# cscott/compressjs

Measured on NVIDIA H100. Metric: bzip2_-9_encode_MBps, higher is better.
Workload: dtype u8

## Files before the change

compressjs_b200/csrc/rle1.cu:

```cuda
#include <algorithm>
#include <cstdlib>
#include "enc.h"

#define RT_THREADS 256
#define RT_PER 16

struct TileSum {
  u32 lead, trail, rest;
  u8 fc, lc, allsame, pad;
};

__host__ __device__ __forceinline__ u64 outfresh(u64 c) {
  u64 q = c / 255, r = c % 255;
  return 5 * q + (r <= 3 ? r : 5);
}
__host__ __device__ __forceinline__ u64 cneed(u64 target) {
  u64 q = (target - 1) / 5, rem = target - 5 * q;
  return 255 * q + (rem <= 3 ? rem : 4);
}
__device__ __forceinline__ u32 w_of_dist(u32 d) {
  u32 r = d % 255 + 1;
  return r <= 3 ? 1u : (r == 4 ? 2u : 0u);
}

struct TileView {
  u8 by[RT_PER];
  u8 w[RT_PER];
  u32 cnt;
  u32 excl;
  u32 total;
  u32 first_start;
  u32 last_start;
  u32 len;
};

struct TileScratch {
  u32 ws[RT_THREADS / 32 + 1];
  u8 lastb[RT_THREADS];
  u32 red[RT_THREADS / 32];
};

__device__ __forceinline__ u32 block_excl_max256(u32 v, u32* ws) {
  u32 inc = warp_incl_max(v);
  u32 exw = __shfl_up_sync(FULL_MASK, inc, 1);
  if (lane_id() == 0) exw = 0;
  const int w = threadIdx.x >> 5;
  if (lane_id() == 31) ws[w] = inc;
  __syncthreads();
  if (w == 0) {
    u32 x = (lane_id() < RT_THREADS / 32) ? ws[lane_id()] : 0u;
    u32 xi = warp_incl_max(x);
    u32 xe = __shfl_up_sync(FULL_MASK, xi, 1);
    if (lane_id() == 0) xe = 0;
    if (lane_id() < RT_THREADS / 32) ws[lane_id()] = xe;
  }
  __syncthreads();
  u32 c = ws[w];
  __syncthreads();
  return exw > c ? exw : c;
}
__device__ __forceinline__ u32 block_min256(u32 v, u32* red) {
#pragma unroll
  for (int o = 16; o > 0; o >>= 1) v = min(v, __shfl_xor_sync(FULL_MASK, v, o));
  if (lane_id() == 0) red[threadIdx.x >> 5] = v;
  __syncthreads();
  u32 r = red[0];
#pragma unroll
  for (int i = 1; i < RT_THREADS / 32; i++) r = min(r, red[i]);
  __syncthreads();
  return r;
}
__device__ __forceinline__ u32 block_max256(u32 v, u32* red) {
#pragma unroll
  for (int o = 16; o > 0; o >>= 1) v = max(v, __shfl_xor_sync(FULL_MASK, v, o));
  if (lane_id() == 0) red[threadIdx.x >> 5] = v;
  __syncthreads();
  u32 r = red[0];
#pragma unroll
  for (int i = 1; i < RT_THREADS / 32; i++) r = max(r, red[i]);
  __syncthreads();
  return r;
}

__device__ void tile_view(const u8* __restrict__ in, u64 N, u64 tstart, u32 carry, TileScratch& sc, TileView& v) {
  const u32 tid = threadIdx.x;
  const u64 remain = N - tstart;
  v.len = remain < RLE_TILE ? (u32)remain : RLE_TILE;
  const u32 pos0 = tid * RT_PER;
  v.cnt = pos0 >= v.len ? 0 : min((u32)RT_PER, v.len - pos0);
  const u8* p = in + tstart + pos0;
  if (v.cnt == RT_PER && (((size_t)p) & 15) == 0) {
    uint4 q = *reinterpret_cast<const uint4*>(p);
    u32 a[4] = {q.x, q.y, q.z, q.w};
#pragma unroll
    for (int j = 0; j < RT_PER; j++) v.by[j] = (u8)(a[j >> 2] >> ((j & 3) * 8));
  } else {
#pragma unroll
    for (int j = 0; j < RT_PER; j++) v.by[j] = (j < (int)v.cnt) ? p[j] : 0;
  }
  sc.lastb[tid] = v.by[RT_PER - 1];
  __syncthreads();
  const u8 prev0 = tid ? sc.lastb[tid - 1] : 0;
  u32 smask = 0, last_local = 0, first_local = 0xffffffffu;
#pragma unroll
  for (int j = 0; j < RT_PER; j++) {
    if (j < (int)v.cnt) {
      const u32 pos = pos0 + j;
      const u8 pb = j ? v.by[j - 1] : prev0;
      const bool st = (pos == 0) || (v.by[j] != pb);
      if (st) {
        smask |= 1u << j;
        last_local = pos + 1;
        if (pos > 0 && first_local == 0xffffffffu) first_local = pos;
      }
    }
  }
  const u32 ex = block_excl_max256(last_local, sc.ws);
  u32 rs = ex ? ex - 1 : 0;
  u32 sum = 0;
#pragma unroll
  for (int j = 0; j < RT_PER; j++) {
    u32 ww = 0;
    if (j < (int)v.cnt) {
      const u32 pos = pos0 + j;
      if (smask & (1u << j)) rs = pos;
      const u32 d = pos - rs + (rs == 0 ? carry : 0);
      ww = w_of_dist(d);
    }
    v.w[j] = (u8)ww;
    sum += ww;
  }
  u32 total;
  v.excl = block_excl_add<RT_THREADS, u32>(sum, sc.ws, &total);
  v.total = total;
  u32 fs = block_min256(first_local, sc.red);
  v.first_start = fs == 0xffffffffu ? v.len : fs;
  u32 ls = block_max256(last_local, sc.red);
  v.last_start = ls ? ls - 1 : 0;
}

__global__ void __launch_bounds__(RT_THREADS) k_rle_summary(const u8* __restrict__ in, u64 N, TileSum* __restrict__ sums, u8* __restrict__ plain) {
  __shared__ TileScratch sc;
  __shared__ u32 lastw[RT_THREADS];
  const u64 t = blockIdx.x;
  const u64 tstart = t * RLE_TILE;
  const u32 tid = threadIdx.x;
  const u64 remain = N - tstart;
  const u32 len = remain < RLE_TILE ? (u32)remain : RLE_TILE;
  const u8* p = in + tstart + tid * RT_PER;
  if (len == RLE_TILE && ((((size_t)in) + tstart) & 15) == 0) {
    const uint4 q = *reinterpret_cast<const uint4*>(p);
    lastw[tid] = q.w;
    __syncthreads();
    u32 prevw;
    if (tid) prevw = lastw[tid - 1];
    else if (tstart >= 4) prevw = ((u32)in[tstart - 1] << 24) | ((u32)in[tstart - 2] << 16) | ((u32)in[tstart - 3] << 8);
    else {
      prevw = 0;
      for (int k = 1; k <= 3; k++) {
        const u32 b = (tstart >= (u64)k) ? in[tstart - k] : (u32)((u8)(~q.x) + k);
        prevw |= b << (8 * (4 - k));
      }
    }
    const u32 a[5] = {prevw, q.x, q.y, q.z, q.w};
    u32 any4 = 0;
#pragma unroll
    for (int wv = 1; wv < 5; wv++) {
      const u32 cur = a[wv], sh1 = __funnelshift_l(a[wv - 1], cur, 8);
      const u32 sh2 = __funnelshift_l(a[wv - 1], cur, 16), sh3 = __funnelshift_l(a[wv - 1], cur, 24);
      const u32 e = __vcmpeq4(cur, sh1) & __vcmpeq4(cur, sh2) & __vcmpeq4(cur, sh3);
      any4 |= e;
    }
    if (!__syncthreads_or(any4 != 0)) {
      if (tid == 0) {
        TileSum s;
        s.fc = in[tstart];
        s.lc = in[tstart + len - 1];
        u32 lead = 1;
        while (lead < 4 && in[tstart + lead] == s.fc) lead++;
        u32 trail = 1;
        while (trail < 4 && in[tstart + len - 1 - trail] == s.lc) trail++;
        s.lead = lead; s.trail = trail; s.allsame = 0; s.rest = len - lead; s.pad = 0;
        sums[t] = s;
        plain[t] = 1;
      }
      return;
    }
  }
  TileView v;
  tile_view(in, N, tstart, 0, sc, v);
  if (threadIdx.x == 0) {
    plain[t] = 0;
    TileSum s;
    s.fc = in[tstart];
    s.lc = in[tstart + v.len - 1];
    s.lead = v.first_start;
    s.allsame = v.first_start == v.len;
    s.trail = v.len - v.last_start;
    s.rest = v.total - (u32)outfresh(v.first_start);
    s.pad = 0;
    sums[t] = s;
  }
}

__device__ __forceinline__ u64 rs_make(bool allsame, u32 fc, u32 lc, u32 trail, u32 len) {
  return (1ull << 63) | ((u64)allsame << 62) | ((u64)fc << 24) | ((u64)lc << 16) | ((u64)trail << 8) | (u64)len;
}
__device__ __forceinline__ u64 rs_combine(u64 A, u64 B) {
  if (!(A >> 63)) return B;
  if (!(B >> 63)) return A;
  const bool Aall = (A >> 62) & 1, Ball = (B >> 62) & 1;
  const u32 Afc = (A >> 24) & 255, Alc = (A >> 16) & 255, Atr = (A >> 8) & 255, Alen = A & 255;
  const u32 Bfc = (B >> 24) & 255, Blc = (B >> 16) & 255, Btr = (B >> 8) & 255, Blen = B & 255;
  const bool join = Alc == Bfc;
  const u32 trail = (Ball && join) ? (Atr + Blen) % 255 : Btr;
  return rs_make(Aall && Ball && join, Afc, Blc, trail, (Alen + Blen) % 255);
}

#define RS_THREADS 1024
__global__ void __launch_bounds__(RS_THREADS)
k_rle_scan(const TileSum* __restrict__ sums, u64 ntiles, u64 N, u32* __restrict__ carry, u64* __restrict__ prefix, u64 st0, u64 W0,
           u64* __restrict__ agg_out) {
  __shared__ u64 sa[RS_THREADS], sb[RS_THREADS];
  const u32 tid = threadIdx.x;
  const u64 per = (ntiles + RS_THREADS - 1) / RS_THREADS;
  const u64 t0 = (u64)tid * per, t1 = min(ntiles, t0 + per);
  u64 agg = 0;
  for (u64 t = t0; t < t1; t++) {
    const TileSum s = sums[t];
    const u64 tl = min((u64)RLE_TILE, N - t * RLE_TILE);
    agg = rs_combine(agg, rs_make(s.allsame, s.fc, s.lc, s.trail % 255, (u32)(tl % 255)));
  }
  sa[tid] = agg;
  __syncthreads();
  u64* src = sa; u64* dst = sb;
  for (u32 o = 1; o < RS_THREADS; o <<= 1) {
    u64 x = src[tid];
    if (tid >= o) x = rs_combine(src[tid - o], x);
    dst[tid] = x;
    __syncthreads();
    u64* tmp = src; src = dst; dst = tmp;
  }
  u64 st = rs_combine(st0, tid ? src[tid - 1] : 0);
  if (tid == 0 && agg_out) *agg_out = src[RS_THREADS - 1];
  __syncthreads();
  u64 mysum = 0;
  for (u64 t = t0; t < t1; t++) {
    const TileSum s = sums[t];
    const u64 tl = min((u64)RLE_TILE, N - t * RLE_TILE);
    u32 c = 0;
    if ((st >> 63) && ((st >> 16) & 255) == s.fc) c = (st >> 8) & 255;
    carry[t] = c;
    const u64 S = outfresh((u64)c + s.lead) - outfresh(c) + s.rest;
    prefix[t] = S;
    mysum += S;
    st = rs_combine(st, rs_make(s.allsame, s.fc, s.lc, s.trail % 255, (u32)(tl % 255)));
  }
  sa[tid] = mysum;
  __syncthreads();
  src = sa; dst = sb;
  for (u32 o = 1; o < RS_THREADS; o <<= 1) {
    u64 x = src[tid];
    if (tid >= o) x += src[tid - o];
    dst[tid] = x;
    __syncthreads();
    u64* tmp = src; src = dst; dst = tmp;
  }
  u64 run = W0 + (tid ? src[tid - 1] : 0);
  const u64 grand = W0 + src[RS_THREADS - 1];
  for (u64 t = t0; t < t1; t++) {
    const u64 S = prefix[t];
    prefix[t] = run;
    run += S;
  }
  if (tid == 0) prefix[ntiles] = grand;
}

#define RG_THREADS 256
#define RG_PER 8
#define RG_TILES (RG_THREADS * RG_PER)
__device__ __forceinline__ u64 rg_tile_state(const TileSum& s, u64 t, u64 N) {
  const u64 tl = min((u64)RLE_TILE, N - t * RLE_TILE);
  return rs_make(s.allsame, s.fc, s.lc, s.trail % 255, (u32)(tl % 255));
}
__device__ __forceinline__ u64 rg_block_excl_state(u64 v, u64* sa, u64* sb, u64* total) {
  const u32 tid = threadIdx.x;
  sa[tid] = v;
  __syncthreads();
  u64* src = sa; u64* dst = sb;
  for (u32 o = 1; o < RG_THREADS; o <<= 1) {
    u64 x = src[tid];
    if (tid >= o) x = rs_combine(src[tid - o], x);
    dst[tid] = x;
    __syncthreads();
    u64* tmp = src; src = dst; dst = tmp;
  }
  const u64 ex = tid ? src[tid - 1] : 0;
  *total = src[RG_THREADS - 1];
  __syncthreads();
  return ex;
}
__global__ void __launch_bounds__(RG_THREADS)
k_rle_scan_g1(const TileSum* __restrict__ sums, u64 ntiles, u64 N, u64* __restrict__ group_agg) {
  __shared__ u64 sa[RG_THREADS], sb[RG_THREADS];
  const u64 t0 = (u64)blockIdx.x * RG_TILES + (u64)threadIdx.x * RG_PER;
  u64 agg = 0;
  for (u32 j = 0; j < RG_PER; j++) {
    const u64 t = t0 + j;
    if (t < ntiles) agg = rs_combine(agg, rg_tile_state(sums[t], t, N));
  }
  u64 total;
  rg_block_excl_state(agg, sa, sb, &total);
  if (threadIdx.x == 0) group_agg[blockIdx.x] = total;
}
template <bool STATE>
__global__ void __launch_bounds__(RS_THREADS)
k_rle_scan_groups(const u64* __restrict__ in, u32 ngroups, u64* __restrict__ out, u64 init, u64* __restrict__ agg_out) {
  __shared__ u64 sa[RS_THREADS], sb[RS_THREADS];
  const u32 tid = threadIdx.x;
  const u32 per = (ngroups + RS_THREADS - 1) / RS_THREADS;
  const u32 g0 = tid * per, g1 = min(ngroups, g0 + per);
  u64 agg = 0;
  for (u32 g = g0; g < g1; g++) agg = STATE ? rs_combine(agg, in[g]) : agg + in[g];
  sa[tid] = agg;
  __syncthreads();
  u64* src = sa; u64* dst = sb;
  for (u32 o = 1; o < RS_THREADS; o <<= 1) {
    u64 x = src[tid];
    if (tid >= o) x = STATE ? rs_combine(src[tid - o], x) : src[tid - o] + x;
    dst[tid] = x;
    __syncthreads();
    u64* tmp = src; src = dst; dst = tmp;
  }
  u64 run = tid ? src[tid - 1] : 0;
  run = STATE ? rs_combine(init, run) : init + run;
  if (tid == 0 && agg_out) *agg_out = src[RS_THREADS - 1];
  for (u32 g = g0; g < g1; g++) {
    const u64 v = in[g];
    out[g] = run;
    run = STATE ? rs_combine(run, v) : run + v;
  }
  if (tid == RS_THREADS - 1) out[ngroups] = STATE ? rs_combine(init, src[RS_THREADS - 1]) : init + src[RS_THREADS - 1];
}
__global__ void __launch_bounds__(RG_THREADS)
k_rle_scan_g3(const TileSum* __restrict__ sums, u64 ntiles, u64 N, const u64* __restrict__ group_start, u32* __restrict__ carry,
              u64* __restrict__ prefix, u64* __restrict__ group_sum) {
  __shared__ u64 sa[RG_THREADS], sb[RG_THREADS];
  __shared__ u32 ws[RG_THREADS / 32 + 1];
  const u64 t0 = (u64)blockIdx.x * RG_TILES + (u64)threadIdx.x * RG_PER;
  TileSum ts[RG_PER];
  u64 agg = 0;
#pragma unroll
  for (u32 j = 0; j < RG_PER; j++) {
    const u64 t = t0 + j;
    if (t < ntiles) { ts[j] = sums[t]; agg = rs_combine(agg, rg_tile_state(ts[j], t, N)); }
  }
  u64 total;
  u64 st = rs_combine(group_start[blockIdx.x], rg_block_excl_state(agg, sa, sb, &total));
  u32 mysum = 0;
#pragma unroll
  for (u32 j = 0; j < RG_PER; j++) {
    const u64 t = t0 + j;
    if (t < ntiles) {
      const TileSum& s = ts[j];
      u32 c = 0;
      if ((st >> 63) && ((st >> 16) & 255) == s.fc) c = (st >> 8) & 255;
      carry[t] = c;
      const u64 S = outfresh((u64)c + s.lead) - outfresh(c) + s.rest;
      prefix[t] = S;
      mysum += (u32)S;
      st = rs_combine(st, rg_tile_state(s, t, N));
    }
  }
  u32 tot;
  block_excl_add<RG_THREADS, u32>(mysum, ws, &tot);
  if (threadIdx.x == 0) group_sum[blockIdx.x] = tot;
}
__global__ void __launch_bounds__(RG_THREADS)
k_rle_scan_g5(u64 ntiles, const u64* __restrict__ group_base, u32 ngroups, u64* __restrict__ prefix) {
  __shared__ u32 ws[RG_THREADS / 32 + 1];
  const u64 t0 = (u64)blockIdx.x * RG_TILES + (u64)threadIdx.x * RG_PER;
  u32 S[RG_PER];
  u32 mysum = 0;
#pragma unroll
  for (u32 j = 0; j < RG_PER; j++) {
    const u64 t = t0 + j;
    S[j] = t < ntiles ? (u32)prefix[t] : 0u;
    mysum += S[j];
  }
  u32 tot;
  u64 run = group_base[blockIdx.x] + block_excl_add<RG_THREADS, u32>(mysum, ws, &tot);
#pragma unroll
  for (u32 j = 0; j < RG_PER; j++) {
    const u64 t = t0 + j;
    if (t < ntiles) { prefix[t] = run; run += S[j]; }
  }
  if (blockIdx.x == 0 && threadIdx.x == 0) prefix[ntiles] = group_base[ngroups];
}

struct BlocksShared {
  TileScratch sc;
  u64 r64;
  u32 r32;
};

__device__ u64 eval_W(const u8* in, u64 N, const u32* carry, const u64* prefix, u64 x, BlocksShared& sh) {
  const u64 t = x / RLE_TILE;
  const u32 off = (u32)(x % RLE_TILE);
  if (off == 0) return prefix[t];
  TileView v;
  tile_view(in, N, t * RLE_TILE, carry[t], sh.sc, v);
  const u32 tid = threadIdx.x;
  if (off / RT_PER == tid) {
    u32 a = v.excl;
    for (u32 j = 0; j < off % RT_PER; j++) a += v.w[j];
    sh.r64 = prefix[t] + a;
  }
  __syncthreads();
  u64 r = sh.r64;
  __syncthreads();
  return r;
}

__device__ u64 find_run_end(const u8* in, u64 s, u64 cap, BlocksShared& sh) {
  const u8 ch = in[s];
  for (u64 base = s; base < cap; base += RLE_TILE) {
    const u64 p0 = base + (u64)threadIdx.x * RT_PER;
    u32 found = 0xffffffffu;
    for (u32 j = 0; j < RT_PER; j++) {
      const u64 p = p0 + j;
      if (p < cap && in[p] != ch) { found = (u32)(p - base); break; }
    }
    const u32 f = block_min256(found, sh.sc.red);
    if (f != 0xffffffffu) return base + f;
  }
  return cap;
}

__global__ void __launch_bounds__(RT_THREADS)
k_rle_blocks(const u8* __restrict__ in, u64 N, u32 BS, const u32* __restrict__ carry, const u64* __restrict__ prefix, u64 ntiles,
             BlkInfo* __restrict__ blocks, u32* nblocks_out, u32 maxblocks, u64 u_start, u32 range_first, u32 range_count, int open_end) {
  __shared__ BlocksShared sh;
  const u32 tid = threadIdx.x;
  const u64 Wtotal = prefix[ntiles];
  if (gridDim.x > 1) {
    const u32 P = gridDim.x, r = blockIdx.x;
    const u32 first = range_first + (u32)((u64)r * range_count / P), next = range_first + (u32)((u64)(r + 1) * range_count / P);
    u_start = (u64)first * BS;
    blocks += first - range_first;
    nblocks_out += r;
    maxblocks = (r == P - 1 && open_end) ? maxblocks - (first - range_first) : next - first;
  }
  u64 s = 0, Ws = prefix[0];
  bool Ws_valid = true;
  u32 k = 0;
  if (u_start > 0) {
    if (u_start > Wtotal) { if (tid == 0) *nblocks_out = 0; return; }
    u64 lo = 0, hi = ntiles;
    while (hi - lo > 1) {
      const u64 span = hi - lo;
      const u64 pi = lo + 1 + (span - 1) * (u64)tid / RT_THREADS;
      const bool valid = pi < hi && (tid == 0 || pi != lo + 1 + (span - 1) * (u64)(tid - 1) / RT_THREADS);
      const bool pr = valid && prefix[pi] < u_start;
      const u32 tr = block_max256(pr ? tid + 1 : 0, sh.sc.red);
      const u32 fl = block_min256((valid && !pr) ? tid : 0xffffffffu, sh.sc.red);
      u64 nlo = lo, nhi = hi;
      if (tr) nlo = lo + 1 + (span - 1) * (u64)(tr - 1) / RT_THREADS;
      if (fl != 0xffffffffu) nhi = lo + 1 + (span - 1) * (u64)fl / RT_THREADS;
      lo = nlo; hi = nhi;
    }
    const u64 t = lo;
    TileView v;
    tile_view(in, N, t * RLE_TILE, carry[t], sh.sc, v);
    u32 found = 0xffffffffu;
    {
      u64 acc = prefix[t] + v.excl;
      for (u32 j = 0; j < v.cnt; j++) {
        acc += v.w[j];
        if (acc >= u_start) { found = tid * RT_PER + j; break; }
      }
    }
    const u32 f = block_min256(found, sh.sc.red);
    if (f / RT_PER == tid) {
      u64 acc = prefix[t] + v.excl;
      for (u32 j = 0; j <= f % RT_PER; j++) acc += v.w[j];
      sh.r64 = acc;
    }
    __syncthreads();
    Ws = sh.r64;
    __syncthreads();
    s = t * RLE_TILE + f + 1;
    Ws_valid = true;
  }
  while (s < N && k < maxblocks) {
    BlkInfo bi;
    bi.s = s;
    const bool midrun = s > 0 && in[s - 1] == in[s];
    u64 b = s;
    if (midrun) {
      const u64 cap = min(N, s + cneed(BS));
      b = find_run_end(in, s, cap, sh);
    }
    const u64 ofs = outfresh(b - s);
    u64 e;
    if (ofs >= BS) {
      e = s + cneed(BS);
      bi.e = e; bi.b = e; bi.Wb = 0; bi.ofs = 0; bi.n = BS;
      Ws_valid = false;
    } else {
      u64 Wb;
      if (midrun) Wb = eval_W(in, N, carry, prefix, b, sh);
      else Wb = Ws_valid ? Ws : eval_W(in, N, carry, prefix, s, sh);
      const u64 V = Wb + (BS - ofs);
      if (V > Wtotal) {
        e = N;
        bi.e = e; bi.b = b; bi.Wb = Wb; bi.ofs = (u32)ofs; bi.n = (u32)(ofs + (Wtotal - Wb));
        Ws_valid = false;
      } else {
        u64 lo = b / RLE_TILE, hi = ntiles;
        {
          const u64 plo = prefix[lo];
          u64 tg = lo + ((V - plo) >> 12);
          if (tg >= ntiles) tg = ntiles - 1;
          const u64 pg = prefix[tg], pg1 = prefix[tg + 1];
          if (pg < V && pg1 >= V) { lo = tg; hi = tg + 1; }
          else if (pg < V) lo = tg;
          else if (tg > lo) hi = tg;
        }
        if (hi - lo > 1) {
          const u64 a = ((BS - ofs) * 4 / 5) / RLE_TILE;
          const u64 g0 = lo + (a > 1 ? a - 1 : 0);
          if (g0 < ntiles && prefix[g0] < V) {
            lo = g0;
            const u64 g1 = g0 + 4 * RT_THREADS;
            if (g1 < ntiles && !(prefix[g1] < V)) hi = g1;
          }
        }
        while (hi - lo > 1) {
          const u64 span = hi - lo;
          const u64 pi = lo + 1 + (span - 1) * (u64)tid / RT_THREADS;
          const bool valid = pi < hi && (tid == 0 || pi != lo + 1 + (span - 1) * (u64)(tid - 1) / RT_THREADS);
          const bool pr = valid && prefix[pi] < V;
          const u32 tr = block_max256(pr ? tid + 1 : 0, sh.sc.red);
          const u32 fl = block_min256((valid && !pr) ? tid : 0xffffffffu, sh.sc.red);
          u64 nlo = lo, nhi = hi;
          if (tr) nlo = lo + 1 + (span - 1) * (u64)(tr - 1) / RT_THREADS;
          if (fl != 0xffffffffu) nhi = lo + 1 + (span - 1) * (u64)fl / RT_THREADS;
          lo = nlo; hi = nhi;
        }
        const u64 t = lo;
        TileView v;
        tile_view(in, N, t * RLE_TILE, carry[t], sh.sc, v);
        u32 found = 0xffffffffu;
        {
          u64 acc = prefix[t] + v.excl;
          for (u32 j = 0; j < v.cnt; j++) {
            acc += v.w[j];
            if (acc >= V) { found = tid * RT_PER + j; break; }
          }
        }
        const u32 f = block_min256(found, sh.sc.red);
        if (f / RT_PER == tid) {
          u64 acc = prefix[t] + v.excl;
          for (u32 j = 0; j <= f % RT_PER; j++) acc += v.w[j];
          sh.r64 = acc;
        }
        __syncthreads();
        const u64 We = sh.r64;
        __syncthreads();
        e = t * RLE_TILE + f + 1;
        const u64 produced = ofs + (We - Wb);
        bi.e = e; bi.b = b; bi.Wb = Wb; bi.ofs = (u32)ofs; bi.n = (u32)min(produced, (u64)BS);
        Ws = We; Ws_valid = true;
      }
    }
    if (tid == 0) blocks[k] = bi;
    k++;
    s = e;
  }
  if (tid == 0) *nblocks_out = k;
}

__global__ void __launch_bounds__(RT_THREADS)
k_rle_emit(const u8* __restrict__ in, u64 N, const u32* __restrict__ carry, const u64* __restrict__ prefix, const u8* __restrict__ plain,
           const BlkInfo* __restrict__ blocks, u32 first, u32 count, const u64* __restrict__ tile_base, u8* __restrict__ T) {
  __shared__ TileScratch sc;
  __shared__ u32 s_k;
  __shared__ __align__(16) u8 stage[RLE_TILE + 32];
  if (threadIdx.x == 0) {
    u32 lo = 0, hi = count;
    while (hi - lo > 1) {
      u32 mid = (lo + hi) >> 1;
      if (tile_base[mid] <= blockIdx.x) lo = mid; else hi = mid;
    }
    s_k = lo;
  }
  __syncthreads();
  const u32 kk = s_k;
  const BlkInfo bi = blocks[first + kk];
  const u64 t = bi.s / RLE_TILE + (blockIdx.x - tile_base[kk]);
  const u64 tstart = t * RLE_TILE;
  u8* Tb = T + ((size_t)kk << SEG_SHIFT);
  const u64 Pt = prefix[t];
  if (plain[t]) {
    const u64 remain = N - tstart;
    const u32 len = remain < RLE_TILE ? (u32)remain : RLE_TILE;
    const u64 x0 = bi.s > tstart ? bi.s : tstart;
    const u64 x1 = (bi.e < tstart + len) ? bi.e : tstart + len;
    if (x0 >= x1) return;
    const u64 o0 = x0 < bi.b ? (x0 - bi.s) : (u64)bi.ofs + (Pt + (x0 - tstart) - bi.Wb);
    if (o0 >= bi.n) return;
    const u32 cnt = (u32)min((u64)(x1 - x0), (u64)bi.n - o0);
    const u32 fo = (u32)(o0 & 15u);
    const u8* src = in + x0;
    for (u32 i = threadIdx.x * 16u; i < cnt; i += RT_THREADS * 16u) {
      if (i + 16u <= cnt && ((((size_t)src) + i) & 15u) == 0) {
        const uint4 q = *reinterpret_cast<const uint4*>(src + i);
        const u32 a[4] = {q.x, q.y, q.z, q.w};
#pragma unroll
        for (int j = 0; j < 16; j++) stage[fo + i + j] = (u8)(a[j >> 2] >> ((j & 3) * 8));
      } else {
        const u32 e = min(i + 16u, cnt);
        for (u32 x = i; x < e; x++) stage[fo + x] = src[x];
      }
    }
    __syncthreads();
    const u32 last = fo + cnt;
    u8* dst = Tb + (o0 - fo);
    for (u32 c16 = threadIdx.x * 16u; c16 < last; c16 += RT_THREADS * 16u) {
      if (c16 >= fo && c16 + 16u <= last) *reinterpret_cast<uint4*>(dst + c16) = *reinterpret_cast<const uint4*>(stage + c16);
      else {
        const u32 e = min(c16 + 16u, last);
        for (u32 x = max(c16, fo); x < e; x++) dst[x] = stage[x];
      }
    }
    return;
  }
  TileView v;
  tile_view(in, N, tstart, carry[t], sc, v);
  u32 run = v.excl;
  for (u32 j = 0; j < v.cnt; j++) {
    const u64 x = tstart + threadIdx.x * RT_PER + j;
    const u32 wmax = v.w[j];
    const u32 exw = run;
    run += wmax;
    if (x < bi.s || x >= bi.e) continue;
    u32 r;
    u64 opos;
    if (x < bi.b) {
      const u64 d = x - bi.s;
      r = (u32)(d % 255) + 1;
      opos = outfresh(d);
    } else {
      r = wmax == 0 ? 5u : (wmax == 2 ? 4u : 1u);
      opos = bi.ofs + (Pt + exw - bi.Wb);
    }
    if (r > 4 || opos >= bi.n) continue;
    const u8 ch = v.by[j];
    Tb[opos] = ch;
    if (r == 4 && opos + 1 < bi.n) {
      u64 lim = x + 1 + 251;
      if (lim > bi.e) lim = bi.e;
      if (x < bi.b && lim > bi.b) lim = bi.b;
      u32 c = 0;
      while (x + 1 + c < lim && in[x + 1 + c] == ch) c++;
      Tb[opos + 1] = (u8)c;
    }
  }
}

#define CRC_POLY 0x04c11db7u
__host__ __device__ __forceinline__ u32 gf_mulmod(u32 a, u32 b) {
  u32 r = 0;
  for (int i = 31; i >= 0; i--) {
    r = (r << 1) ^ ((r & 0x80000000u) ? CRC_POLY : 0u);
    if ((b >> i) & 1) r ^= a;
  }
  return r;
}
struct CrcConsts {
  u32 table[256];
  u32 pow[48];
  u32 slice[3][256];
};
static CrcConsts make_crc_consts() {
  CrcConsts c;
  for (u32 i = 0; i < 256; i++) {
    u32 v = i << 24;
    for (int k = 0; k < 8; k++) v = (v & 0x80000000u) ? (v << 1) ^ CRC_POLY : (v << 1);
    c.table[i] = v;
  }
  for (int k = 0; k < 3; k++)
    for (u32 i = 0; i < 256; i++) {
      const u32 prev = k ? c.slice[k - 1][i] : c.table[i];
      c.slice[k][i] = (prev << 8) ^ c.table[prev >> 24];
    }
  c.pow[0] = 0x100;
  for (int i = 1; i < 48; i++) c.pow[i] = gf_mulmod(c.pow[i - 1], c.pow[i - 1]);
  return c;
}
__constant__ CrcConsts c_crc;
static bool g_crc_ready = false;
static void crc_setup() {
  if (g_crc_ready) return;
  CrcConsts h = make_crc_consts();
  CUDA_CHECK(cudaMemcpyToSymbol(c_crc, &h, sizeof h));
  g_crc_ready = true;
}
__device__ __forceinline__ u32 crc_xpow(u64 bytes) {
  u32 r = 1u;
  for (int i = 0; bytes; i++, bytes >>= 1)
    if (bytes & 1) r = gf_mulmod(r, c_crc.pow[i]);
  return r;
}

#define CRC_PIECE 256
__host__ __device__ __forceinline__ u64 crc_piece_count(u64 s, u64 e, u32 mis) {
  return e > s ? (e - 1 + mis) / CRC_PIECE - (s + mis) / CRC_PIECE + 1 : 0;
}
__global__ void __launch_bounds__(256)
k_crc_pieces(const u8* __restrict__ in, const BlkInfo* __restrict__ blocks, u32 first, u32 count, const u64* __restrict__ piece_base,
             u64 total_pieces, u32* __restrict__ acc) {
  __shared__ u32 tab[256], t1[256], t2[256], t3[256];
  tab[threadIdx.x] = c_crc.table[threadIdx.x];
  t1[threadIdx.x] = c_crc.slice[0][threadIdx.x];
  t2[threadIdx.x] = c_crc.slice[1][threadIdx.x];
  t3[threadIdx.x] = c_crc.slice[2][threadIdx.x];
  __syncthreads();
  const u64 gid = (u64)blockIdx.x * blockDim.x + threadIdx.x;
  if (gid >= total_pieces) return;
  u32 lo = 0, hi = count;
  while (hi - lo > 1) {
    u32 mid = (lo + hi) >> 1;
    if (piece_base[mid] <= gid) lo = mid; else hi = mid;
  }
  const BlkInfo bi = blocks[first + lo];
  const u32 mis = (u32)((size_t)in & (CRC_PIECE - 1));
  const u64 j = gid - piece_base[lo];
  const u64 A = ((bi.s + mis) / CRC_PIECE + j) * CRC_PIECE;
  const u64 pbeg = A > bi.s + mis ? A - mis : bi.s;
  const u64 pend = A + CRC_PIECE < bi.e + mis ? A + CRC_PIECE - mis : bi.e;
  u32 crc = 0;
  const u8* p = in + pbeg;
  const u32 len = (u32)(pend - pbeg);
  if (len == CRC_PIECE) {
    for (u32 i = 0; i < CRC_PIECE; i += 16) {
      uint4 q = *reinterpret_cast<const uint4*>(p + i);
      u32 a[4] = {q.x, q.y, q.z, q.w};
#pragma unroll
      for (int w = 0; w < 4; w++) {
        const u32 x = crc ^ __byte_perm(a[w], 0, 0x0123);
        crc = t3[x >> 24] ^ t2[(x >> 16) & 0xff] ^ t1[(x >> 8) & 0xff] ^ tab[x & 0xff];
      }
    }
  } else {
    for (u32 i = 0; i < len; i++) crc = (crc << 8) ^ tab[((crc >> 24) ^ p[i]) & 0xff];
  }
  if (pend == bi.e) {
    atomicXor(&acc[2 * lo + 1], crc);
  } else {
    const u64 k = (bi.e - pend) / CRC_PIECE;
    if (k) crc = gf_mulmod(crc, crc_xpow(k * CRC_PIECE));
    atomicXor(&acc[2 * lo], crc);
  }
}
__global__ void k_crc_final(const u8* __restrict__ in, const BlkInfo* __restrict__ blocks, u32 first, u32 count, const u32* __restrict__ acc,
                            u32* __restrict__ crc_out) {
  u32 k = blockIdx.x * blockDim.x + threadIdx.x;
  if (k >= count) return;
  const BlkInfo bi = blocks[first + k];
  const u64 len = bi.e - bi.s;
  const u32 mis = (u32)((size_t)in & (CRC_PIECE - 1));
  const u32 body = gf_mulmod(acc[2 * k], crc_xpow((bi.e + mis) % CRC_PIECE)) ^ acc[2 * k + 1];
  crc_out[k] = ~(body ^ gf_mulmod(0xffffffffu, crc_xpow(len)));
}

u32 crc32_device(Ctx& c, const u8* d_p, size_t n) {
  crc_setup();
  BlkInfo bi;
  memset(&bi, 0, sizeof bi);
  bi.s = 0; bi.e = n; bi.b = 0; bi.n = 0;
  DBuf<BlkInfo> db(c, 1);
  DBuf<u64> pb(c, 1);
  DBuf<u32> acc(c, 2), out(c, 1);
  u64 zero = 0;
  c.to_device(db, &bi, sizeof bi);
  c.to_device(pb, &zero, 8);
  CUDA_CHECK(cudaMemsetAsync(acc, 0, 8, c.stream));
  const u64 pieces = crc_piece_count(0, n, (u32)((size_t)d_p & (CRC_PIECE - 1)));
  if (pieces) {
    k_crc_pieces<<<(unsigned)((pieces + 255) / 256), 256, 0, c.stream>>>(d_p, db, 0, 1, pb, pieces, acc);
    KLAUNCH(c); KCHECK();
  }
  k_crc_final<<<1, 32, 0, c.stream>>>(d_p, db, 0, 1, acc, out);
  KLAUNCH(c); KCHECK();
  u32 h = 0;
  c.to_host(&h, out, 4);
  c.sync();
  return h;
}

__global__ void k_share_lead(const TileSum* __restrict__ sums, u64 ntiles, u64* __restrict__ out) {
  if (threadIdx.x) return;
  u64 lead = 0;
  const u8 fc = sums[0].fc;
  for (u64 t = 0; t < ntiles; t++) {
    const TileSum s = sums[t];
    if (s.fc != fc) break;
    lead += s.lead;
    if (!s.allsame) break;
  }
  *out = lead;
}

void rle1_scan_tiles(Ctx& c, const u8* d_in, size_t n, Rle1Plan& plan, u64 st0, u64 W0, u64* summary) {
  crc_setup();
  StageScope s(c, ST_RLE1);
  if (n == 0) return;
  const u64 ntiles = (n + RLE_TILE - 1) / RLE_TILE;
  DBuf<TileSum> sums(c, ntiles);
  DBuf<u64> dagg(c, 4);
  plan.tile_carry.alloc(c, ntiles);
  plan.tile_prefix.alloc(c, ntiles + 1);
  plan.tile_plain.alloc(c, ntiles);
  k_rle_summary<<<(unsigned)ntiles, RT_THREADS, 0, c.stream>>>(d_in, n, sums, plan.tile_plain);
  KLAUNCH(c); KCHECK();
  static const bool force_groups = getenv("B2_RLE_SCAN_GROUPS") != nullptr;
  if (ntiles <= 4 * RG_TILES && !force_groups) {
    k_rle_scan<<<1, RS_THREADS, 0, c.stream>>>(sums, ntiles, n, plan.tile_carry, plan.tile_prefix, st0, W0, dagg);
    KLAUNCH(c); KCHECK();
  } else {
    c.stats.rle_group_scans++;
    const u32 ng = (u32)((ntiles + RG_TILES - 1) / RG_TILES);
    DBuf<u64> gagg(c, ng), gstart(c, ng + 1), gsum(c, ng), gbase(c, ng + 1);
    k_rle_scan_g1<<<ng, RG_THREADS, 0, c.stream>>>(sums, ntiles, n, gagg);
    KLAUNCH(c); KCHECK();
    k_rle_scan_groups<true><<<1, RS_THREADS, 0, c.stream>>>(gagg, ng, gstart, st0, dagg);
    KLAUNCH(c); KCHECK();
    k_rle_scan_g3<<<ng, RG_THREADS, 0, c.stream>>>(sums, ntiles, n, gstart, plan.tile_carry, plan.tile_prefix, gsum);
    KLAUNCH(c); KCHECK();
    k_rle_scan_groups<false><<<1, RS_THREADS, 0, c.stream>>>(gsum, ng, gbase, W0, nullptr);
    KLAUNCH(c); KCHECK();
    k_rle_scan_g5<<<ng, RG_THREADS, 0, c.stream>>>(ntiles, gbase, ng, plan.tile_prefix);
    KLAUNCH(c); KCHECK();
  }
  if (summary) {
    k_share_lead<<<1, 32, 0, c.stream>>>(sums, ntiles, dagg.p + 1);
    KLAUNCH(c); KCHECK();
    c.to_host(summary, dagg, 16);
  }
  c.to_host(&plan.w_total, plan.tile_prefix.p + ntiles, 8);
  c.sync();
}

static void cut_blocks(Ctx& c, const u8* d_in, size_t n, int level, Rle1Plan& plan, bool exact, size_t first, size_t count) {
  StageScope s(c, ST_RLE1);
  if (n == 0) return;
  const u32 BS = rle1_block_size(level);
  const u64 ntiles = (n + RLE_TILE - 1) / RLE_TILE;
  u32 maxblocks = (u32)(n / ((u64)BS * 4 / 5) + 2);
  u64 u_start = 0;
  if (!exact) {
    maxblocks = (u32)std::min<size_t>(maxblocks, count);
    u_start = (u64)first * BS;
    plan.first_index = first;
    if (maxblocks == 0) return;
  }
  plan.blocks.alloc(c, maxblocks);
  const u32 total = (u32)plan.total_guess(level);
  const u32 rfirst = exact ? 0u : (u32)first, rcount = exact ? total : maxblocks;
  const u32 P = std::min<u32>(64, rcount / 8);
  if (P > 1 && (!exact || total < maxblocks)) {
    DBuf<u32> dnb(c, P);
    k_rle_blocks<<<P, RT_THREADS, 0, c.stream>>>(d_in, n, BS, plan.tile_carry, plan.tile_prefix, ntiles, plan.blocks, dnb, maxblocks, 0, rfirst, rcount,
                                                exact ? 1 : 0);
    KLAUNCH(c); KCHECK();
    std::vector<u32> cut(P);
    c.to_host(cut.data(), dnb, 4 * P);
    c.sync();
    bool ok = true;
    for (u32 r = 0; r + 1 < P && ok; r++) ok = cut[r] == (u32)((u64)(r + 1) * rcount / P) - (u32)((u64)r * rcount / P);
    const u32 last_first = (u32)((u64)(P - 1) * rcount / P);
    ok = ok && cut[P - 1] > 0;
    if (ok) {
      const u32 nb = last_first + cut[P - 1];
      plan.h_blocks.resize(nb);
      c.to_host(plan.h_blocks.data(), plan.blocks, sizeof(BlkInfo) * nb);
      c.sync();
      ok = !exact || (plan.h_blocks[0].s == 0 && plan.h_blocks[nb - 1].e == n);
      for (u32 k = 0; k + 1 < nb && ok; k++) ok = plan.h_blocks[k].e == plan.h_blocks[k + 1].s;
      if (ok) { plan.nblocks = nb; c.stats.rle_walk_parallel++; return; }
      plan.h_blocks.clear();
    }
  }
  c.stats.rle_walk_serial++;
  DBuf<u32> dnb(c, 1);
  k_rle_blocks<<<1, RT_THREADS, 0, c.stream>>>(d_in, n, BS, plan.tile_carry, plan.tile_prefix, ntiles, plan.blocks, dnb, maxblocks, u_start, 0, 0, 0);
  KLAUNCH(c); KCHECK();
  u32 nb = 0;
  c.to_host(&nb, dnb, 4);
  c.sync();
  plan.nblocks = nb;
  plan.h_blocks.resize(nb);
  if (nb) c.to_host(plan.h_blocks.data(), plan.blocks, sizeof(BlkInfo) * nb);
  c.sync();
}
void rle1_cut_range(Ctx& c, const u8* d_in, size_t n, int level, Rle1Plan& plan, size_t first, size_t count) {
  cut_blocks(c, d_in, n, level, plan, false, first, count);
}
void rle1_plan(Ctx& c, const u8* d_in, size_t n, int level, Rle1Plan& plan) {
  rle1_scan_tiles(c, d_in, n, plan);
  cut_blocks(c, d_in, n, level, plan, true, 0, 0);
}
void rle1_materialize(Ctx& c, const u8* d_in, size_t n, const Rle1Plan& plan, size_t first, size_t count, u8* d_T, u32* d_n, u32* d_crc) {
  if (count == 0) return;
  std::vector<u64> tbase(count + 1), pbase(count + 1);
  std::vector<u32> hn(count);
  u64 tt = 0, pp = 0;
  for (size_t k = 0; k < count; k++) {
    const BlkInfo& bi = plan.h_blocks[first + k];
    tbase[k] = tt; pbase[k] = pp;
    tt += (bi.e - 1) / RLE_TILE - bi.s / RLE_TILE + 1;
    pp += crc_piece_count(bi.s, bi.e, (u32)((size_t)d_in & (CRC_PIECE - 1)));
    hn[k] = bi.n;
  }
  tbase[count] = tt; pbase[count] = pp;
  DBuf<u64> dtb(c, count + 1), dpb(c, count + 1);
  DBuf<u32> acc(c, 2 * count);
  c.to_device(dtb, tbase.data(), 8 * (count + 1));
  c.to_device(dpb, pbase.data(), 8 * (count + 1));
  c.to_device(d_n, hn.data(), 4 * count);
  CUDA_CHECK(cudaMemsetAsync(acc, 0, 8 * count, c.stream));
  k_rle_emit<<<(unsigned)tt, RT_THREADS, 0, c.stream>>>(d_in, n, plan.tile_carry, plan.tile_prefix, plan.tile_plain, plan.blocks, (u32)first, (u32)count, dtb, d_T);
  KLAUNCH(c); KCHECK();
  k_crc_pieces<<<(unsigned)((pp + 255) / 256), 256, 0, c.stream>>>(d_in, plan.blocks, (u32)first, (u32)count, dpb, pp, acc);
  KLAUNCH(c); KCHECK();
  k_crc_final<<<(unsigned)((count + 127) / 128), 128, 0, c.stream>>>(d_in, plan.blocks, (u32)first, (u32)count, acc, d_crc);
  KLAUNCH(c); KCHECK();
}

void crc_ranges(Ctx& c, const u8* d_data, const BlkInfo* d_ranges, const std::vector<BlkInfo>& h_ranges, u32* d_crc_out) {
  crc_setup();
  const size_t count = h_ranges.size();
  if (count == 0) return;
  std::vector<u64> pbase(count + 1);
  u64 pp = 0;
  for (size_t k = 0; k < count; k++) {
    pbase[k] = pp;
    pp += crc_piece_count(h_ranges[k].s, h_ranges[k].e, (u32)((size_t)d_data & (CRC_PIECE - 1)));
  }
  pbase[count] = pp;
  DBuf<u64> dpb(c, count + 1);
  DBuf<u32> acc(c, 2 * count);
  c.to_device(dpb, pbase.data(), 8 * (count + 1));
  CUDA_CHECK(cudaMemsetAsync(acc, 0, 8 * count, c.stream));
  if (pp) {
    k_crc_pieces<<<(unsigned)((pp + 255) / 256), 256, 0, c.stream>>>(d_data, d_ranges, 0, (u32)count, dpb, pp, acc);
    KLAUNCH(c); KCHECK();
  }
  k_crc_final<<<(unsigned)((count + 127) / 128), 128, 0, c.stream>>>(d_data, d_ranges, 0, (u32)count, acc, d_crc_out);
  KLAUNCH(c); KCHECK();
  c.sync();
}
```

Before: 25340.

## Fuse block CRC into RLE1 emit kernel with multi-tile spans

The RLE1 emit kernel now handles four tiles per CTA, stages the input bytes in swizzled shared memory, and computes the block CRC from that staged data using segment CRCs combined through precomputed GF(2) power tables. This replaces the separate k_crc_pieces pass over the input, and the device-side binary search is replaced by a precomputed block/span map. The cost is a larger constant table in global memory, an extra small map kernel, more shared memory per CTA, and a hard limit on block length.

```diff
diff --git a/compressjs_b200/csrc/rle1.cu b/compressjs_b200/csrc/rle1.cu
--- a/compressjs_b200/csrc/rle1.cu
+++ b/compressjs_b200/csrc/rle1.cu
@@ -581,63 +581,112 @@
   if (tid == 0) *nblocks_out = k;
 }
 
-__global__ void __launch_bounds__(RT_THREADS)
-k_rle_emit(const u8* __restrict__ in, u64 N, const u32* __restrict__ carry, const u64* __restrict__ prefix, const u8* __restrict__ plain,
-           const BlkInfo* __restrict__ blocks, u32 first, u32 count, const u64* __restrict__ tile_base, u8* __restrict__ T) {
-  __shared__ TileScratch sc;
-  __shared__ u32 s_k;
-  __shared__ __align__(16) u8 stage[RLE_TILE + 32];
-  if (threadIdx.x == 0) {
-    u32 lo = 0, hi = count;
-    while (hi - lo > 1) {
-      u32 mid = (lo + hi) >> 1;
-      if (tile_base[mid] <= blockIdx.x) lo = mid; else hi = mid;
-    }
-    s_k = lo;
-  }
-  __syncthreads();
-  const u32 kk = s_k;
-  const BlkInfo bi = blocks[first + kk];
-  const u64 t = bi.s / RLE_TILE + (blockIdx.x - tile_base[kk]);
-  const u64 tstart = t * RLE_TILE;
-  u8* Tb = T + ((size_t)kk << SEG_SHIFT);
-  const u64 Pt = prefix[t];
-  if (plain[t]) {
-    const u64 remain = N - tstart;
-    const u32 len = remain < RLE_TILE ? (u32)remain : RLE_TILE;
-    const u64 x0 = bi.s > tstart ? bi.s : tstart;
-    const u64 x1 = (bi.e < tstart + len) ? bi.e : tstart + len;
-    if (x0 >= x1) return;
-    const u64 o0 = x0 < bi.b ? (x0 - bi.s) : (u64)bi.ofs + (Pt + (x0 - tstart) - bi.Wb);
-    if (o0 >= bi.n) return;
-    const u32 cnt = (u32)min((u64)(x1 - x0), (u64)bi.n - o0);
-    const u32 fo = (u32)(o0 & 15u);
-    const u8* src = in + x0;
-    for (u32 i = threadIdx.x * 16u; i < cnt; i += RT_THREADS * 16u) {
-      if (i + 16u <= cnt && ((((size_t)src) + i) & 15u) == 0) {
-        const uint4 q = *reinterpret_cast<const uint4*>(src + i);
-        const u32 a[4] = {q.x, q.y, q.z, q.w};
-#pragma unroll
-        for (int j = 0; j < 16; j++) stage[fo + i + j] = (u8)(a[j >> 2] >> ((j & 3) * 8));
-      } else {
-        const u32 e = min(i + 16u, cnt);
-        for (u32 x = i; x < e; x++) stage[fo + x] = src[x];
-      }
-    }
-    __syncthreads();
-    const u32 last = fo + cnt;
-    u8* dst = Tb + (o0 - fo);
-    for (u32 c16 = threadIdx.x * 16u; c16 < last; c16 += RT_THREADS * 16u) {
-      if (c16 >= fo && c16 + 16u <= last) *reinterpret_cast<uint4*>(dst + c16) = *reinterpret_cast<const uint4*>(stage + c16);
-      else {
-        const u32 e = min(c16 + 16u, last);
-        for (u32 x = max(c16, fo); x < e; x++) dst[x] = stage[x];
-      }
-    }
-    return;
-  }
-  TileView v;
-  tile_view(in, N, tstart, carry[t], sc, v);
+#define CRC_POLY 0x04c11db7u
+__host__ __device__ __forceinline__ u32 gf_mulmod(u32 a, u32 b) {
+  u32 r = 0;
+  for (int i = 31; i >= 0; i--) {
+    r = (r << 1) ^ ((r & 0x80000000u) ? CRC_POLY : 0u);
+    if ((b >> i) & 1) r ^= a;
+  }
+  return r;
+}
+#define EMIT_TILES 4
+#define EMIT_SPAN (EMIT_TILES * RLE_TILE)
+#define EMIT_SEG 64
+static_assert(EMIT_SEG * RT_THREADS == EMIT_SPAN, "every emit thread takes one segment of the span");
+#define CRC_TILE_POWS 11264
+struct CrcConsts {
+  u32 slice[4][256];
+  u32 pow[48];
+  u32 pow_byte[EMIT_SEG + 1];
+  u32 pow_seg[EMIT_SPAN / EMIT_SEG];
+  u32 pow_tile[CRC_TILE_POWS];
+};
+static void make_crc_consts(CrcConsts& c) {
+  for (u32 i = 0; i < 256; i++) {
+    u32 v = i << 24;
+    for (int k = 0; k < 8; k++) v = (v & 0x80000000u) ? (v << 1) ^ CRC_POLY : (v << 1);
+    c.slice[0][i] = v;
+  }
+  for (int k = 1; k < 4; k++)
+    for (u32 i = 0; i < 256; i++) {
+      const u32 prev = c.slice[k - 1][i];
+      c.slice[k][i] = (prev << 8) ^ c.slice[0][prev >> 24];
+    }
+  c.pow[0] = 0x100;
+  for (int i = 1; i < 48; i++) c.pow[i] = gf_mulmod(c.pow[i - 1], c.pow[i - 1]);
+  c.pow_byte[0] = 1u;
+  for (int r = 1; r <= EMIT_SEG; r++) c.pow_byte[r] = gf_mulmod(c.pow_byte[r - 1], c.pow[0]);
+  c.pow_seg[0] = 1u;
+  for (int m = 1; m < EMIT_SPAN / EMIT_SEG; m++) c.pow_seg[m] = gf_mulmod(c.pow_seg[m - 1], c.pow_byte[EMIT_SEG]);
+  const u32 xtile = c.pow[12];
+  c.pow_tile[0] = 1u;
+  for (int k = 1; k < CRC_TILE_POWS; k++) c.pow_tile[k] = gf_mulmod(c.pow_tile[k - 1], xtile);
+}
+static_assert(RLE_TILE == 1 << 12, "pow_tile is built from pow[12]");
+__device__ CrcConsts g_crc;
+static bool g_crc_ready = false;
+static void crc_setup() {
+  if (g_crc_ready) return;
+  static CrcConsts h;
+  make_crc_consts(h);
+  CUDA_CHECK(cudaMemcpyToSymbol(g_crc, &h, sizeof h));
+  g_crc_ready = true;
+}
+__device__ __forceinline__ u32 crc_xpow(u64 bytes) {
+  u32 r = 1u;
+  for (int i = 0; bytes; i++, bytes >>= 1)
+    if (bytes & 1) r = gf_mulmod(r, g_crc.pow[i]);
+  return r;
+}
+__device__ __forceinline__ void crc_load_tables(u32 (*tab)[256]) {
+#pragma unroll
+  for (int k = 0; k < 4; k++) tab[k][threadIdx.x] = g_crc.slice[k][threadIdx.x];
+}
+__device__ __forceinline__ u32 crc_step4(u32 crc, u32 w, const u32 (*tab)[256]) {
+  const u32 x = crc ^ __byte_perm(w, 0, 0x0123);
+  return tab[3][x >> 24] ^ tab[2][(x >> 16) & 0xff] ^ tab[1][(x >> 8) & 0xff] ^ tab[0][x & 0xff];
+}
+__device__ __forceinline__ u32 crc_step1(u32 crc, u32 byte, const u32 (*tab)[256]) { return (crc << 8) ^ tab[0][((crc >> 24) ^ byte) & 0xff]; }
+
+#define EMIT_STAGE_WORDS (EMIT_SPAN / 16 + 16)
+__device__ __forceinline__ u32 emit_sw(int w) {
+  const u32 v = (u32)(w + 8);
+  return v ^ ((v >> 3) & 3);
+}
+__device__ __forceinline__ u32 stage_byte(const uint4* stage, u32 p) {
+  return reinterpret_cast<const u8*>(stage)[16 * emit_sw((int)(p >> 4)) + (p & 15)];
+}
+__device__ __forceinline__ uint4 load16(const u8* __restrict__ in, u64 N, u64 off) {
+  const u8* p = in + off;
+  if (off + 16 <= N && (((size_t)p) & 15) == 0) return *reinterpret_cast<const uint4*>(p);
+  u32 a[4] = {0, 0, 0, 0};
+  for (u32 j = 0; j < 16 && off + j < N; j++) a[j >> 2] |= (u32)p[j] << (8 * (j & 3));
+  return make_uint4(a[0], a[1], a[2], a[3]);
+}
+__device__ void emit_copy(const uint4* stage, u32 ra, u64 o0, u32 cnt, u8* __restrict__ Tb) {
+  const u32 fo = (u32)(o0 & 15u);
+  const int delta = (int)ra - (int)fo;
+  const int wq = delta >> 4;
+  const u32 sh = (u32)delta & 15u, q = sh >> 2, bs = 8 * (sh & 3);
+  const u32 end = fo + cnt, nw = (end + 15) >> 4;
+  u8* dst = Tb + (o0 - fo);
+  for (u32 k = threadIdx.x; k < nw; k += RT_THREADS) {
+    const u32 b0 = 16 * k;
+    if (b0 >= fo && b0 + 16 <= end) {
+      const uint4 lo = stage[emit_sw(wq + (int)k)], hi = stage[emit_sw(wq + (int)k + 1)];
+      const u32 a[8] = {lo.x, lo.y, lo.z, lo.w, hi.x, hi.y, hi.z, hi.w};
+      u32 b[5];
+#pragma unroll
+      for (int j = 0; j < 5; j++) b[j] = q == 0 ? a[j] : q == 1 ? a[j + 1] : q == 2 ? a[j + 2] : a[j + 3];
+      *reinterpret_cast<uint4*>(dst + b0) = make_uint4(__funnelshift_r(b[0], b[1], bs), __funnelshift_r(b[1], b[2], bs),
+                                                       __funnelshift_r(b[2], b[3], bs), __funnelshift_r(b[3], b[4], bs));
+    } else {
+      for (u32 x = max(b0, fo); x < min(b0 + 16, end); x++) dst[x] = (u8)stage_byte(stage, (u32)(delta + (int)x));
+    }
+  }
+}
+__device__ void emit_general(const u8* __restrict__ in, const BlkInfo& bi, u64 tstart, u64 Pt, const TileView& v, u8* __restrict__ Tb) {
   u32 run = v.excl;
   for (u32 j = 0; j < v.cnt; j++) {
     const u64 x = tstart + threadIdx.x * RT_PER + j;
@@ -668,50 +717,98 @@
     }
   }
 }
-
-#define CRC_POLY 0x04c11db7u
-__host__ __device__ __forceinline__ u32 gf_mulmod(u32 a, u32 b) {
-  u32 r = 0;
-  for (int i = 31; i >= 0; i--) {
-    r = (r << 1) ^ ((r & 0x80000000u) ? CRC_POLY : 0u);
-    if ((b >> i) & 1) r ^= a;
-  }
-  return r;
-}
-struct CrcConsts {
-  u32 table[256];
-  u32 pow[48];
-  u32 slice[3][256];
-};
-static CrcConsts make_crc_consts() {
-  CrcConsts c;
-  for (u32 i = 0; i < 256; i++) {
-    u32 v = i << 24;
-    for (int k = 0; k < 8; k++) v = (v & 0x80000000u) ? (v << 1) ^ CRC_POLY : (v << 1);
-    c.table[i] = v;
-  }
-  for (int k = 0; k < 3; k++)
-    for (u32 i = 0; i < 256; i++) {
-      const u32 prev = k ? c.slice[k - 1][i] : c.table[i];
-      c.slice[k][i] = (prev << 8) ^ c.table[prev >> 24];
-    }
-  c.pow[0] = 0x100;
-  for (int i = 1; i < 48; i++) c.pow[i] = gf_mulmod(c.pow[i - 1], c.pow[i - 1]);
-  return c;
-}
-__constant__ CrcConsts c_crc;
-static bool g_crc_ready = false;
-static void crc_setup() {
-  if (g_crc_ready) return;
-  CrcConsts h = make_crc_consts();
-  CUDA_CHECK(cudaMemcpyToSymbol(c_crc, &h, sizeof h));
-  g_crc_ready = true;
-}
-__device__ __forceinline__ u32 crc_xpow(u64 bytes) {
-  u32 r = 1u;
-  for (int i = 0; bytes; i++, bytes >>= 1)
-    if (bytes & 1) r = gf_mulmod(r, c_crc.pow[i]);
-  return r;
+__global__ void __launch_bounds__(RT_THREADS, 6)
+k_rle_emit(const u8* __restrict__ in, u64 N, const u32* __restrict__ carry, const u64* __restrict__ prefix, const u8* __restrict__ plain,
+           const BlkInfo* __restrict__ blocks, u32 first, const uint2* __restrict__ map, u8* __restrict__ T, u32* __restrict__ acc) {
+  __shared__ __align__(16) uint4 stage[EMIT_STAGE_WORDS];
+  __shared__ u32 tab[4][256];
+  __shared__ TileScratch sc;
+  __shared__ u32 red[RT_THREADS / 32 + 1];
+  const u32 tid = threadIdx.x;
+  crc_load_tables(tab);
+  const uint2 m = map[blockIdx.x];
+  const BlkInfo bi = blocks[first + m.x];
+  const u64 t0 = bi.s / RLE_TILE + (u64)m.y * EMIT_TILES;
+  const u32 ntl = (u32)min((u64)EMIT_TILES, (bi.e - 1) / RLE_TILE - t0 + 1);
+  const u64 sstart = t0 * RLE_TILE;
+  const u64 X0 = max(bi.s, sstart), X1 = min(bi.e, sstart + (u64)ntl * RLE_TILE);
+  u8* Tb = T + ((size_t)m.x << SEG_SHIFT);
+  u32 pmask = 0;
+#pragma unroll
+  for (u32 i = 0; i < EMIT_TILES; i++)
+    if (i < ntl && plain[t0 + i]) pmask |= 1u << i;
+  uint4 q[EMIT_TILES];
+#pragma unroll
+  for (u32 i = 0; i < EMIT_TILES; i++)
+    if ((pmask >> i) & 1) q[i] = load16(in, N, sstart + i * RLE_TILE + 16 * tid);
+#pragma unroll
+  for (u32 i = 0; i < EMIT_TILES; i++)
+    if ((pmask >> i) & 1) stage[emit_sw((int)(i * RT_THREADS + tid))] = q[i];
+  for (u32 i = 0; i < ntl; i++) {
+    if ((pmask >> i) & 1) continue;
+    const u64 t = t0 + i, tstart = t * RLE_TILE;
+    TileView v;
+    tile_view(in, N, tstart, carry[t], sc, v);
+    emit_general(in, bi, tstart, prefix[t], v, Tb);
+    u32 a[4] = {0, 0, 0, 0};
+#pragma unroll
+    for (int j = 0; j < RT_PER; j++) a[j >> 2] |= (u32)v.by[j] << (8 * (j & 3));
+    stage[emit_sw((int)(i * RT_THREADS + tid))] = make_uint4(a[0], a[1], a[2], a[3]);
+  }
+  __syncthreads();
+  for (u32 i = 0; i < ntl;) {
+    if (!((pmask >> i) & 1)) { i++; continue; }
+    u32 j = i + 1;
+    while (j < ntl && ((pmask >> j) & 1)) j++;
+    const u64 tstart = sstart + (u64)i * RLE_TILE;
+    const u64 x0 = max(X0, tstart), x1 = min(X1, sstart + (u64)j * RLE_TILE);
+    const u64 o0 = x0 < bi.b ? (x0 - bi.s) : (u64)bi.ofs + (prefix[t0 + i] + (x0 - tstart) - bi.Wb);
+    if (o0 < bi.n) emit_copy(stage, (u32)(x0 - sstart), o0, (u32)min(x1 - x0, (u64)bi.n - o0), Tb);
+    i = j;
+  }
+  const u32 rx0 = (u32)(X0 - sstart), rx1 = (u32)(X1 - sstart);
+  const u32 seg0 = tid * EMIT_SEG;
+  u32 R = 0;
+  if (seg0 < rx1 && seg0 + EMIT_SEG > rx0) {
+#pragma unroll
+    for (u32 j4 = 0; j4 < EMIT_SEG / 16; j4++) {
+      const uint4 s4 = stage[emit_sw((int)(tid * (EMIT_SEG / 16) + j4))];
+      const u32 a[4] = {s4.x, s4.y, s4.z, s4.w};
+#pragma unroll
+      for (u32 w = 0; w < 4; w++) {
+        const u32 pos = seg0 + 16 * j4 + 4 * w;
+        u32 x = a[w];
+        if (pos < rx0) x = rx0 - pos >= 4 ? 0u : x & (0xffffffffu << (8 * (rx0 - pos)));
+        if (pos + 4 <= rx1) R = crc_step4(R, x, tab);
+        else
+          for (u32 b = pos; b < rx1; b++) R = crc_step1(R, x >> (8 * (b - pos)), tab);
+      }
+    }
+  }
+  const u32 L = (rx1 - 1) / EMIT_SEG, r = rx1 - L * EMIT_SEG;
+  u32 c = tid < L ? gf_mulmod(R, g_crc.pow_seg[L - 1 - tid]) : 0u;
+#pragma unroll
+  for (int o = 16; o > 0; o >>= 1) c ^= __shfl_xor_sync(FULL_MASK, c, o);
+  if (lane_id() == 0) red[tid >> 5] = c;
+  if (tid == L) red[RT_THREADS / 32] = R;
+  __syncthreads();
+  if (tid == 0) {
+    u32 S = 0;
+#pragma unroll
+    for (int w = 0; w < RT_THREADS / 32; w++) S ^= red[w];
+    u32 tot = gf_mulmod(S, g_crc.pow_byte[r]) ^ red[RT_THREADS / 32];
+    if (X1 == bi.e) {
+      atomicXor(&acc[2 * m.x + 1], tot);
+    } else {
+      const u64 k = bi.e / RLE_TILE - X1 / RLE_TILE;
+      if (k) tot = gf_mulmod(tot, g_crc.pow_tile[k]);
+      atomicXor(&acc[2 * m.x], tot);
+    }
+  }
+}
+__global__ void k_emit_map(const u32* __restrict__ sbase, uint2* __restrict__ map) {
+  const u32 k = blockIdx.x, b = sbase[k], n = sbase[k + 1] - b;
+  for (u32 j = threadIdx.x; j < n; j += blockDim.x) map[b + j] = make_uint2(k, j);
 }
 
 #define CRC_PIECE 256
@@ -721,11 +818,8 @@
 __global__ void __launch_bounds__(256)
 k_crc_pieces(const u8* __restrict__ in, const BlkInfo* __restrict__ blocks, u32 first, u32 count, const u64* __restrict__ piece_base,
              u64 total_pieces, u32* __restrict__ acc) {
-  __shared__ u32 tab[256], t1[256], t2[256], t3[256];
-  tab[threadIdx.x] = c_crc.table[threadIdx.x];
-  t1[threadIdx.x] = c_crc.slice[0][threadIdx.x];
-  t2[threadIdx.x] = c_crc.slice[1][threadIdx.x];
-  t3[threadIdx.x] = c_crc.slice[2][threadIdx.x];
+  __shared__ u32 tab[4][256];
+  crc_load_tables(tab);
   __syncthreads();
   const u64 gid = (u64)blockIdx.x * blockDim.x + threadIdx.x;
   if (gid >= total_pieces) return;
@@ -746,15 +840,13 @@
   if (len == CRC_PIECE) {
     for (u32 i = 0; i < CRC_PIECE; i += 16) {
       uint4 q = *reinterpret_cast<const uint4*>(p + i);
-      u32 a[4] = {q.x, q.y, q.z, q.w};
-#pragma unroll
-      for (int w = 0; w < 4; w++) {
-        const u32 x = crc ^ __byte_perm(a[w], 0, 0x0123);
-        crc = t3[x >> 24] ^ t2[(x >> 16) & 0xff] ^ t1[(x >> 8) & 0xff] ^ tab[x & 0xff];
-      }
+      crc = crc_step4(crc, q.x, tab);
+      crc = crc_step4(crc, q.y, tab);
+      crc = crc_step4(crc, q.z, tab);
+      crc = crc_step4(crc, q.w, tab);
     }
   } else {
-    for (u32 i = 0; i < len; i++) crc = (crc << 8) ^ tab[((crc >> 24) ^ p[i]) & 0xff];
+    for (u32 i = 0; i < len; i++) crc = crc_step1(crc, p[i], tab);
   }
   if (pend == bi.e) {
     atomicXor(&acc[2 * lo + 1], crc);
@@ -764,14 +856,13 @@
     atomicXor(&acc[2 * lo], crc);
   }
 }
-__global__ void k_crc_final(const u8* __restrict__ in, const BlkInfo* __restrict__ blocks, u32 first, u32 count, const u32* __restrict__ acc,
+__global__ void k_crc_final(const BlkInfo* __restrict__ blocks, u32 first, u32 count, const u32* __restrict__ acc, u32 unit, u32 mis,
                             u32* __restrict__ crc_out) {
   u32 k = blockIdx.x * blockDim.x + threadIdx.x;
   if (k >= count) return;
   const BlkInfo bi = blocks[first + k];
   const u64 len = bi.e - bi.s;
-  const u32 mis = (u32)((size_t)in & (CRC_PIECE - 1));
-  const u32 body = gf_mulmod(acc[2 * k], crc_xpow((bi.e + mis) % CRC_PIECE)) ^ acc[2 * k + 1];
+  const u32 body = gf_mulmod(acc[2 * k], crc_xpow((bi.e + mis) % unit)) ^ acc[2 * k + 1];
   crc_out[k] = ~(body ^ gf_mulmod(0xffffffffu, crc_xpow(len)));
 }
 
@@ -787,12 +878,13 @@
   c.to_device(db, &bi, sizeof bi);
   c.to_device(pb, &zero, 8);
   CUDA_CHECK(cudaMemsetAsync(acc, 0, 8, c.stream));
-  const u64 pieces = crc_piece_count(0, n, (u32)((size_t)d_p & (CRC_PIECE - 1)));
+  const u32 mis = (u32)((size_t)d_p & (CRC_PIECE - 1));
+  const u64 pieces = crc_piece_count(0, n, mis);
   if (pieces) {
     k_crc_pieces<<<(unsigned)((pieces + 255) / 256), 256, 0, c.stream>>>(d_p, db, 0, 1, pb, pieces, acc);
     KLAUNCH(c); KCHECK();
   }
-  k_crc_final<<<1, 32, 0, c.stream>>>(d_p, db, 0, 1, acc, out);
+  k_crc_final<<<1, 32, 0, c.stream>>>(db, 0, 1, acc, CRC_PIECE, mis, out);
   KLAUNCH(c); KCHECK();
   u32 h = 0;
   c.to_host(&h, out, 4);
@@ -914,28 +1006,31 @@
 }
 void rle1_materialize(Ctx& c, const u8* d_in, size_t n, const Rle1Plan& plan, size_t first, size_t count, u8* d_T, u32* d_n, u32* d_crc) {
   if (count == 0) return;
-  std::vector<u64> tbase(count + 1), pbase(count + 1);
+  crc_setup();
+  std::vector<u32> sbase(count + 1);
   std::vector<u32> hn(count);
-  u64 tt = 0, pp = 0;
+  u64 ss = 0;
   for (size_t k = 0; k < count; k++) {
     const BlkInfo& bi = plan.h_blocks[first + k];
-    tbase[k] = tt; pbase[k] = pp;
-    tt += (bi.e - 1) / RLE_TILE - bi.s / RLE_TILE + 1;
-    pp += crc_piece_count(bi.s, bi.e, (u32)((size_t)d_in & (CRC_PIECE - 1)));
+    const u64 ta = bi.s / RLE_TILE, tb = (bi.e - 1) / RLE_TILE;
+    if (bi.e / RLE_TILE - ta >= CRC_TILE_POWS) throw B2Error{B2_ERR_CUDA, "internal error: RLE1 block longer than the CRC shift table"};
+    sbase[k] = (u32)ss;
+    ss += (tb - ta + EMIT_TILES) / EMIT_TILES;
     hn[k] = bi.n;
   }
-  tbase[count] = tt; pbase[count] = pp;
-  DBuf<u64> dtb(c, count + 1), dpb(c, count + 1);
+  sbase[count] = (u32)ss;
+  DBuf<u32> dsb(c, count + 1);
+  DBuf<uint2> map(c, ss);
   DBuf<u32> acc(c, 2 * count);
-  c.to_device(dtb, tbase.data(), 8 * (count + 1));
-  c.to_device(dpb, pbase.data(), 8 * (count + 1));
+  c.to_device(dsb, sbase.data(), 4 * (count + 1));
   c.to_device(d_n, hn.data(), 4 * count);
   CUDA_CHECK(cudaMemsetAsync(acc, 0, 8 * count, c.stream));
-  k_rle_emit<<<(unsigned)tt, RT_THREADS, 0, c.stream>>>(d_in, n, plan.tile_carry, plan.tile_prefix, plan.tile_plain, plan.blocks, (u32)first, (u32)count, dtb, d_T);
+  k_emit_map<<<(unsigned)count, 128, 0, c.stream>>>(dsb, map);
   KLAUNCH(c); KCHECK();
-  k_crc_pieces<<<(unsigned)((pp + 255) / 256), 256, 0, c.stream>>>(d_in, plan.blocks, (u32)first, (u32)count, dpb, pp, acc);
+  k_rle_emit<<<(unsigned)ss, RT_THREADS, 0, c.stream>>>(d_in, n, plan.tile_carry, plan.tile_prefix, plan.tile_plain, plan.blocks, (u32)first, map,
+                                                       d_T, acc);
   KLAUNCH(c); KCHECK();
-  k_crc_final<<<(unsigned)((count + 127) / 128), 128, 0, c.stream>>>(d_in, plan.blocks, (u32)first, (u32)count, acc, d_crc);
+  k_crc_final<<<(unsigned)((count + 127) / 128), 128, 0, c.stream>>>(plan.blocks, (u32)first, (u32)count, acc, RLE_TILE, 0, d_crc);
   KLAUNCH(c); KCHECK();
 }
 
@@ -943,11 +1038,12 @@
   crc_setup();
   const size_t count = h_ranges.size();
   if (count == 0) return;
+  const u32 mis = (u32)((size_t)d_data & (CRC_PIECE - 1));
   std::vector<u64> pbase(count + 1);
   u64 pp = 0;
   for (size_t k = 0; k < count; k++) {
     pbase[k] = pp;
-    pp += crc_piece_count(h_ranges[k].s, h_ranges[k].e, (u32)((size_t)d_data & (CRC_PIECE - 1)));
+    pp += crc_piece_count(h_ranges[k].s, h_ranges[k].e, mis);
   }
   pbase[count] = pp;
   DBuf<u64> dpb(c, count + 1);
@@ -958,7 +1054,7 @@
     k_crc_pieces<<<(unsigned)((pp + 255) / 256), 256, 0, c.stream>>>(d_data, d_ranges, 0, (u32)count, dpb, pp, acc);
     KLAUNCH(c); KCHECK();
   }
-  k_crc_final<<<(unsigned)((count + 127) / 128), 128, 0, c.stream>>>(d_data, d_ranges, 0, (u32)count, acc, d_crc_out);
+  k_crc_final<<<(unsigned)((count + 127) / 128), 128, 0, c.stream>>>(d_ranges, 0, (u32)count, acc, CRC_PIECE, mis, d_crc_out);
   KLAUNCH(c); KCHECK();
   c.sync();
 }
```

Result: faster. 26970 (median of 6 runs) (+6.4%).
